# Minys233/GCN-BMP

Hardware: AMD Instinct MI355X
Metric: drug-pairs/sec fwd+bwd, binary-DDI GGNN d=128 (higher is better)
Workload: dtype f32; 1 GPU; C2: full binary DDI set (544 drugs, 147696 pairs), GGNN 4-step d=128 tied + Nie co-attention (head 8, tanh) + MLP(32,16), fwd+bwd+Adam, 1024 pairs/GPU/step, every molecule instance encoded; the 144 batches of one epoch resident in HBM, cycled; layout=per-instance packed layout, whole 128-row tiles, pairs_per_gpu=1024, global_batch=1024, parallelism=dp1

## Files before the change

gcn-bmp_amd/csrc/bmp_coattn.hip:

```cpp
#include <string.h>
#include "bmp_kernels.h"

#define CO_MAXN 128
#define CO_MAXH 16
#define CO_NT_BIG 1024
#define CO_DQ 4
#define CO_NT_FWD 512

struct CoArgs {
    const float* X1; const float* X2;
    const float* Q2;
    const float* Z1; const float* Z2; int ZC;
    const float* w1; const float* w2;
    const int* r1; const int* n1; const int* r2; const int* n2;
    const long long* coff;
    const int* order; int order_off;
    int np;
    const float* wa1; const float* wa2; const float* cbias;
    int d, o, H, act, ldc;
    int mode;
    float* Cbuf;
    float* H1; float* H2;
    float* al1; float* al2;
    float* out1; float* out2;
    const float* dout1; const float* dout2;
    float* dQ2; float* dX1;
    float* dZ1; float* dZ2;
    float* dpart;
    float* big_ws; long long big_stride;
    const int* rm1; const int* rm2; int N1, N2;
    const float* gscale;
};

struct CoLds {
    float* Cs;
    float* dSs;
    float* P1s;
    float* P2s;
    float* dH1s;
    float* dH2s;
    float* w1s; float* w2s; float* v2s;
    float* cmax; float* invD2; float* rmax; float* invD1;
    float* s1; float* s2;
    float* dots1; float* dots2;
    float* H1s; float* H2s;
    float* do1; float* do2;
    float* Up; float* dPp; float* cmb;
};

__device__ __forceinline__ CoLds co_carve(float* base, int np, int ldc, int H, bool bwd, int o = 0, int nt = 256, bool big = false) {
    CoLds L;
    float* p = base;
    L.Cs = p; p += (size_t)np * ldc;
    L.dSs = p; if (bwd) p += (size_t)np * ldc;
    L.P1s = p; p += np * H;
    L.P2s = p; p += np * H;
    L.dH1s = p; if (bwd) p += np * H;
    L.dH2s = p; if (bwd) p += np * H;
    L.w1s = p; p += np;
    L.w2s = p; p += np;
    L.v2s = p; p += np;
    L.cmax = p; p += np; L.invD2 = p; p += np; L.rmax = p; p += np; L.invD1 = p; p += np;
    L.s1 = p; p += np;
    L.s2 = p; p += np;
    L.dots1 = p; p += np; L.dots2 = p; p += np;
    L.H1s = p; if (bwd) p += np * H;
    L.H2s = p; if (bwd) p += np * H;
    L.do1 = p; if (bwd) p += o;
    L.do2 = p; if (bwd) p += o;
    L.cmb = p; if (bwd) p += np;
    if (big) { L.Up = p; if (bwd) p += np; L.dPp = p; if (bwd) p += np * H; }
    else if (np >= 128) { L.Up = L.dots1; L.dPp = L.H1s; }
    else { L.Up = p; if (bwd) p += nt; L.dPp = p; if (bwd) p += nt * H; }
    return L;
}

static size_t co_lds_floats(int np, int ldc, int H, bool bwd, int o = 0, int nt = 256, bool big = false) {
    return (size_t)np * ldc * (bwd ? 2 : 1) + (size_t)np * H * (bwd ? 6 : 2) + 11 * (size_t)np + (bwd ? 2 * (size_t)o + np : 0) +
           (big ? (bwd ? np + np * (size_t)H : 0) : ((bwd && np < 128) ? nt + nt * (size_t)H : 0));
}
static int co_big_np(int np_big) { return (np_big + 31) & ~31; }
static size_t co_big_stride(int np_big, int H, bool bwd, int o) {
    const int np = co_big_np(np_big);
    return (co_lds_floats(np, np + 1, H, bwd, o, 512, true) + 15) & ~(size_t)15;
}

__device__ __forceinline__ void co_stats(const CoLds& L, int n1, int n2, int ldc) {
    const int tid = threadIdx.x;
    if (tid < CO_MAXN) {
        const int j = tid;
        if (j < n1) {
            float mx = -INFINITY;
            for (int i = 0; i < n2; ++i) if (L.w2s[i] > 0.f) mx = fmaxf(mx, L.Cs[i * ldc + j]);
            float s = 0.f;
            for (int i = 0; i < n2; ++i) if (L.w2s[i] > 0.f) s += L.w2s[i] * bmp_exp(L.Cs[i * ldc + j] - mx);
            L.cmax[j] = mx; L.invD2[j] = 1.f / s;
        }
    } else {
        const int i = tid - CO_MAXN;
        if (i < n2) {
            float mx = -INFINITY;
            for (int j = 0; j < n1; ++j) if (L.w1s[j] > 0.f) mx = fmaxf(mx, L.Cs[i * ldc + j]);
            float s = 0.f;
            for (int j = 0; j < n1; ++j) if (L.w1s[j] > 0.f) s += L.w1s[j] * bmp_exp(L.Cs[i * ldc + j] - mx);
            L.rmax[i] = mx; L.invD1[i] = 1.f / s;
        }
    }
}

__device__ __forceinline__ float grp_max(float v, int Q) {
    for (int m = Q >> 1; m >= 1; m >>= 1) v = fmaxf(v, __shfl_xor(v, m));
    return v;
}
__device__ __forceinline__ float grp_sum(float v, int Q) {
    for (int m = Q >> 1; m >= 1; m >>= 1) v += __shfl_xor(v, m);
    return v;
}
__device__ __forceinline__ int co_split(int n1, int n2, int nt) {
    int Q = 1;
    while (Q < 16 && 2 * Q * (n1 + n2) <= nt) Q *= 2;
    return Q;
}
__device__ __forceinline__ void co_stats_split(const CoLds& L, int n1, int n2, int ldc, int Q) {
    const int a = threadIdx.x / Q, q = threadIdx.x % Q;
    if (a < n1) {
        const int j = a;
        float mx = -INFINITY;
        for (int i = q; i < n2; i += Q) if (L.w2s[i] > 0.f) mx = fmaxf(mx, L.Cs[i * ldc + j]);
        mx = grp_max(mx, Q);
        float s = 0.f;
        for (int i = q; i < n2; i += Q) if (L.w2s[i] > 0.f) s += L.w2s[i] * bmp_exp(L.Cs[i * ldc + j] - mx);
        s = grp_sum(s, Q);
        if (q == 0) { L.cmax[j] = mx; L.invD2[j] = 1.f / s; }
    } else if (a < n1 + n2) {
        const int i = a - n1;
        float mx = -INFINITY;
        for (int j = q; j < n1; j += Q) if (L.w1s[j] > 0.f) mx = fmaxf(mx, L.Cs[i * ldc + j]);
        mx = grp_max(mx, Q);
        float s = 0.f;
        for (int j = q; j < n1; j += Q) if (L.w1s[j] > 0.f) s += L.w1s[j] * bmp_exp(L.Cs[i * ldc + j] - mx);
        s = grp_sum(s, Q);
        if (q == 0) { L.rmax[i] = mx; L.invD1[i] = 1.f / s; }
    }
}

__device__ __forceinline__ void co_stats_split_big(const CoLds& L, int n1, int n2, int ldc, int nt) {
    for (int a = threadIdx.x; a < n1 + n2; a += nt) {
        if (a < n1) {
            const int j = a;
            float mx = -INFINITY;
            for (int i = 0; i < n2; ++i) if (L.w2s[i] > 0.f) mx = fmaxf(mx, L.Cs[i * ldc + j]);
            float s = 0.f;
            for (int i = 0; i < n2; ++i) if (L.w2s[i] > 0.f) s += L.w2s[i] * bmp_exp(L.Cs[i * ldc + j] - mx);
            L.cmax[j] = mx; L.invD2[j] = 1.f / s;
        } else {
            const int i = a - n1;
            float mx = -INFINITY;
            for (int j = 0; j < n1; ++j) if (L.w1s[j] > 0.f) mx = fmaxf(mx, L.Cs[i * ldc + j]);
            float s = 0.f;
            for (int j = 0; j < n1; ++j) if (L.w1s[j] > 0.f) s += L.w1s[j] * bmp_exp(L.Cs[i * ldc + j] - mx);
            L.rmax[i] = mx; L.invD1[i] = 1.f / s;
        }
    }
}

__device__ __forceinline__ float co_L2(const CoLds& L, int i, int j, int ldc) {
    return L.w2s[i] > 0.f ? bmp_exp(L.Cs[i * ldc + j] - L.cmax[j]) * L.invD2[j] : 0.f;
}
__device__ __forceinline__ float co_L1(const CoLds& L, int i, int j, int ldc) {
    return L.w1s[j] > 0.f ? bmp_exp(L.Cs[i * ldc + j] - L.rmax[i]) * L.invD1[i] : 0.f;
}

template <int HT, int NT, bool BIG = false>
__global__ __launch_bounds__(NT) void k_coattn_fwd(CoArgs a) {
    constexpr int NW = NT / 64;
    constexpr int HN = HT > 0 ? HT : CO_MAXH;
    extern __shared__ __attribute__((aligned(16))) float lds_raw[];
    const int b = a.order[a.order_off + blockIdx.x];
    const int tid = threadIdx.x, lane = tid & 63, wave = tid >> 6;
    const int l31 = lane & 31, hi = lane >> 5;
    const int r1 = a.r1[b], n1 = a.n1[b], r2 = a.r2[b], n2 = a.n2[b];
    const int d = a.d, o = a.o, H = HT > 0 ? HT : a.H, ZC = a.ZC, ldc = a.ldc;
    const int nb1 = (n1 + 31) >> 5, nb2 = (n2 + 31) >> 5;
    const CoLds L = BIG ? co_carve(a.big_ws + (size_t)blockIdx.x * a.big_stride, a.np, ldc, H, false, 0, NT, true)
                        : co_carve(lds_raw, a.np, ldc, H, false);
    const float cb = a.cbias[0];

    for (int idx = tid; idx < n1 * H; idx += NT) L.P1s[idx] = a.Z1[(size_t)(r1 + idx / H) * ZC + o + idx % H];
    for (int idx = tid; idx < n2 * H; idx += NT) L.P2s[idx] = a.Z2[(size_t)(r2 + idx / H) * ZC + o + idx % H];
    if constexpr (BIG) {
        for (int j = tid; j < n1; j += NT) L.w1s[j] = a.w1[r1 + j];
        for (int i = tid; i < n2; i += NT) { L.w2s[i] = a.w2[r2 + i]; L.v2s[i] = a.Z2[(size_t)(r2 + i) * ZC + o + H]; }
    } else {
    if (tid < n1) L.w1s[tid] = a.w1[r1 + tid];
    if (tid >= CO_MAXN && tid - CO_MAXN < n2) {
        const int i = tid - CO_MAXN;
        L.w2s[i] = a.w2[r2 + i];
        L.v2s[i] = a.Z2[(size_t)(r2 + i) * ZC + o + H];
    }
    }
    __syncthreads();

    for (int blk = wave; blk < nb2 * nb1; blk += NW) {
        const int bi = blk / nb1, bj = blk % nb1;
        int ia = bi * 32 + l31; ia = ia < n2 ? ia : n2 - 1;
        int ja = bj * 32 + l31; ja = ja < n1 ? ja : n1 - 1;
        const float* qa = a.Q2 + (size_t)(r2 + ia) * d + 4 * hi;
        const float* xb = a.X1 + (size_t)(r1 + ja) * d + 4 * hi;
        f32x16 acc;
#pragma unroll
        for (int t = 0; t < 16; ++t) acc[t] = 0.f;
#pragma unroll 8
        for (int k0 = 0; k0 < d; k0 += 8) {
            const f32x4 av = *(const f32x4*)(qa + k0);
            const f32x4 bv = *(const f32x4*)(xb + k0);
#pragma unroll
            for (int t = 0; t < 4; ++t) acc = bmp_mfma(av[t], bv[t], acc);
        }
        const int j = bj * 32 + l31;
        const float v1j = j < n1 ? a.Z1[(size_t)(r1 + j) * ZC + o + H] : 0.f;
        float* cg = a.Cbuf + a.coff[b];
#pragma unroll
        for (int reg = 0; reg < 16; ++reg) {
            const int i = bi * 32 + bmp_acc_row(reg, lane);
            if (i < n2 && j < n1) {
                const float cv = bmp_act(a.act, acc[reg] + v1j + L.v2s[i] + cb);
                L.Cs[i * ldc + j] = cv;
                if (a.Cbuf) cg[(size_t)i * n1 + j] = cv;
            }
        }
    }
    __syncthreads();
    if (a.mode == 1) {
        for (int t_ = tid; t_ < (BIG ? n1 + n2 : NT); t_ += NT) {
        const bool s1 = BIG ? t_ < n1 : t_ < CO_MAXN;
        if (s1) {
            const int j = t_;
            if (j < n1) {
                float s = 0.f, A2 = 0.f;
                for (int i = 0; i < n2; ++i) { s += L.w2s[i] * L.Cs[i * ldc + j]; A2 += L.w2s[i]; }
                L.s1[j] = s / A2;
            }
        } else {
            const int i = t_ - (BIG ? n1 : CO_MAXN);
            if (i < n2) {
                float s = 0.f, A1 = 0.f;
                for (int j = 0; j < n1; ++j) { s += L.w1s[j] * L.Cs[i * ldc + j]; A1 += L.w1s[j]; }
                L.s2[i] = s / A1;
            }
        }
        }
    } else {
    const int Q = BIG ? 1 : co_split(n1, n2, NT);
    if constexpr (BIG) co_stats_split_big(L, n1, n2, ldc, NT);
    else co_stats_split(L, n1, n2, ldc, Q);
    __syncthreads();
    if (a.Cbuf) {
        float* st = a.Cbuf + a.coff[b] + (size_t)n2 * n1;
        if constexpr (BIG) {
            for (int j = tid; j < n1; j += NT) { st[j] = L.cmax[j]; st[n1 + j] = L.invD2[j]; }
            for (int i = tid; i < n2; i += NT) { st[2 * n1 + i] = L.rmax[i]; st[2 * n1 + n2 + i] = L.invD1[i]; }
        } else {
        if (tid < CO_MAXN) { if (tid < n1) { st[tid] = L.cmax[tid]; st[n1 + tid] = L.invD2[tid]; } }
        else if (tid < 2 * CO_MAXN) { const int i = tid - CO_MAXN; if (i < n2) { st[2 * n1 + i] = L.rmax[i]; st[2 * n1 + n2 + i] = L.invD1[i]; } }
        }
    }
    __syncthreads();

    for (int a_ = tid / Q; a_ < (BIG ? n1 + n2 : tid / Q + 1); a_ += NT) {
        const int q = tid % Q;
        const bool side1 = a_ < n1, valid = a_ < n1 + n2;
        const int me = side1 ? a_ : a_ - n1;
        const int no = side1 ? n2 : n1;
        const float* Po = side1 ? L.P2s : L.P1s;
        const float* wo = side1 ? L.w2s : L.w1s;
        float acc[HN];
#pragma unroll
        for (int h = 0; h < HN; ++h) acc[h] = 0.f;
        if (valid) {
            for (int k = q; k < no; k += Q) {
                const float e = wo[k] * (side1 ? co_L1(L, k, me, ldc) : co_L2(L, me, k, ldc));
#pragma unroll
                for (int h = 0; h < HN; ++h) if (h < H) acc[h] += e * Po[k * H + h];
            }
        }
#pragma unroll
        for (int h = 0; h < HN; ++h) if (h < H) acc[h] = grp_sum(acc[h], Q);
        if (valid && q == 0) {
            const float* Pm = side1 ? L.P1s : L.P2s;
            const float* wa = side1 ? a.wa1 : a.wa2;
            float* Hg = a.H1 == nullptr ? nullptr : (side1 ? a.H1 + (size_t)(r1 + me) * H : a.H2 + (size_t)(r2 + me) * H);
            float sc = 0.f;
#pragma unroll
            for (int h = 0; h < HN; ++h) if (h < H) {
                const float hv = bmp_tanh(Pm[me * H + h] + acc[h]);
                if (Hg) Hg[h] = hv;
                sc += hv * wa[h];
            }
            (side1 ? L.s1 : L.s2)[me] = sc;
        }
    }
    }
    __syncthreads();

    if (wave < 2) {
        float* sc = wave == 0 ? L.s1 : L.s2;
        const float* ww = wave == 0 ? L.w1s : L.w2s;
        const int n = wave == 0 ? n1 : n2;
        float mx = -INFINITY;
        for (int k = lane; k < n; k += 64) if (ww[k] > 0.f) mx = fmaxf(mx, sc[k]);
        mx = bmp_wave_max(mx);
        float s = 0.f;
        for (int k = lane; k < n; k += 64) if (ww[k] > 0.f) s += ww[k] * bmp_exp(sc[k] - mx);
        s = bmp_wave_sum(s);
        float* alg = a.al1 == nullptr ? nullptr : (wave == 0 ? a.al1 + r1 : a.al2 + r2);
        for (int k = lane; k < n; k += 64) {
            const float al = ww[k] > 0.f ? bmp_exp(sc[k] - mx) / s : 0.f;
            sc[k] = al;
            if (alg) alg[k] = al;
        }
    }
    __syncthreads();

    {
        constexpr int KG = NT / 256;
        const int kg = tid >> 8, side = (tid >> 7) & 1, t = tid & 127;
        const float* Z = side == 0 ? a.Z1 + (size_t)r1 * ZC : a.Z2 + (size_t)r2 * ZC;
        const float* al = side == 0 ? L.s1 : L.s2;
        const float* ww = side == 0 ? L.w1s : L.w2s;
        const int n = side == 0 ? n1 : n2;
        const int chunk = (n + KG - 1) / KG, k_lo = kg * chunk, k_hi = (k_lo + chunk) < n ? (k_lo + chunk) : n;
        float* out = (side == 0 ? a.out1 : a.out2) + (size_t)b * o;
        float* part = L.Cs;
        for (int c0 = 0; c0 < o; c0 += 128) {
            const int c = c0 + t;
            float acc = 0.f;
            if (c < o) {
#pragma unroll 8
                for (int k = k_lo; k < k_hi; ++k) acc += ww[k] * al[k] * Z[(size_t)k * ZC + c];
            }
            if (KG == 1) {
                if (c < o) out[c] = acc;
            } else {
                __syncthreads();
                part[(kg * 2 + side) * 128 + t] = acc;
                __syncthreads();
                if (kg == 0 && c < o) {
                    float v = part[side * 128 + t];
#pragma unroll
                    for (int g = 1; g < KG; ++g) v += part[(g * 2 + side) * 128 + t];
                    out[c] = v;
                }
            }
        }
    }
}

template <int HT, int NT, bool BIG = false>
__global__ __launch_bounds__(NT) void k_coattn_bwd(CoArgs a) {
    constexpr int NW = NT / 64;
    constexpr int HN = HT > 0 ? HT : CO_MAXH;
    extern __shared__ __attribute__((aligned(16))) float lds_raw[];
    const int b = a.order[a.order_off + blockIdx.x];
    const int tid = threadIdx.x, lane = tid & 63, wave = tid >> 6;
    const int l31 = lane & 31, hi = lane >> 5;
    const int r1 = a.r1[b], n1 = a.n1[b], r2 = a.r2[b], n2 = a.n2[b];
    const int d = a.d, o = a.o, H = HT > 0 ? HT : a.H, ZC = a.ZC, ldc = a.ldc;
    const int nb1 = (n1 + 31) >> 5, nb2 = (n2 + 31) >> 5;
    const int n1p = nb1 * 32, n2p = nb2 * 32;
    const CoLds L = BIG ? co_carve(a.big_ws + (size_t)blockIdx.x * a.big_stride, a.np, ldc, H, true, o, NT, true)
                        : co_carve(lds_raw, a.np, ldc, H, true, o, NT);
    if (a.rm1 != nullptr) {
        for (int row = r1 + n1; row < a.N1 && a.rm1[row] < 0; ++row) {
            for (int c = tid; c < d; c += NT) a.dX1[(size_t)row * d + c] = 0.f;
            for (int c = tid; c < ZC; c += NT) a.dZ1[(size_t)row * ZC + c] = 0.f;
        }
        for (int row = r2 + n2; row < a.N2 && a.rm2[row] < 0; ++row) {
            for (int c = tid; c < d; c += NT) a.dQ2[(size_t)row * d + c] = 0.f;
            for (int c = tid; c < ZC; c += NT) a.dZ2[(size_t)row * ZC + c] = 0.f;
        }
    }
    {
        const float* st = a.Cbuf + a.coff[b] + (size_t)n2 * n1;
        if constexpr (BIG) {
            for (int j = tid; j < n1; j += NT) { L.cmax[j] = st[j]; L.invD2[j] = st[n1 + j]; }
            for (int i = tid; i < n2; i += NT) { L.rmax[i] = st[2 * n1 + i]; L.invD1[i] = st[2 * n1 + n2 + i]; }
        } else {
        if (tid < CO_MAXN) { if (tid < n1) { L.cmax[tid] = st[tid]; L.invD2[tid] = st[n1 + tid]; } }
        else if (tid < 2 * CO_MAXN) { const int i = tid - CO_MAXN; if (i < n2) { L.rmax[i] = st[2 * n1 + i]; L.invD1[i] = st[2 * n1 + n2 + i]; } }
        }
    }
    for (int idx = tid; idx < n1 * H; idx += NT) L.P1s[idx] = a.Z1[(size_t)(r1 + idx / H) * ZC + o + idx % H];
    for (int idx = tid; idx < n2 * H; idx += NT) L.P2s[idx] = a.Z2[(size_t)(r2 + idx / H) * ZC + o + idx % H];
    for (int idx = tid; idx < n1 * H; idx += NT) L.H1s[idx] = a.H1[(size_t)r1 * H + idx];
    for (int idx = tid; idx < n2 * H; idx += NT) L.H2s[idx] = a.H2[(size_t)r2 * H + idx];
    {
        const float gs = a.gscale ? a.gscale[0] : 1.f;
        for (int c = tid; c < o; c += NT) { L.do1[c] = a.dout1[(size_t)b * o + c] * gs; L.do2[c] = a.dout2[(size_t)b * o + c] * gs; }
    }
    if constexpr (BIG) {
        for (int j = tid; j < n1; j += NT) { L.w1s[j] = a.w1[r1 + j]; L.s1[j] = a.al1[r1 + j]; }
        for (int i = tid; i < n2; i += NT) { L.w2s[i] = a.w2[r2 + i]; L.s2[i] = a.al2[r2 + i]; }
    } else {
    if (tid < n1) { L.w1s[tid] = a.w1[r1 + tid]; L.s1[tid] = a.al1[r1 + tid]; }
    if (tid >= CO_MAXN && tid - CO_MAXN < n2) {
        const int i = tid - CO_MAXN;
        L.w2s[i] = a.w2[r2 + i]; L.s2[i] = a.al2[r2 + i];
    }
    }
    {
        const float* cg = a.Cbuf + a.coff[b];
        for (int idx = tid; idx < n2p * ldc; idx += NT) { L.dSs[idx] = 0.f; }
        for (int idx = tid; idx < n2 * n1; idx += NT) L.Cs[(idx / n1) * ldc + idx % n1] = cg[idx];
    }
    const int ncb = (d + 31) >> 5;
    float pre[16];
#pragma unroll
    for (int t = 0; t < 16; ++t) pre[t] = 0.f;
    if (wave < (nb2 + nb1) * ncb) {
        const bool isq = wave < nb2 * ncb;
        const int bc = (isq ? wave : wave - nb2 * ncb) % ncb;
        const int col = bc * 32 + l31;
        const int colc = col < d ? col : d - 1;
        const int kn = isq ? n1 : n2;
        const float* src = isq ? a.X1 + (size_t)r1 * d : a.Q2 + (size_t)r2 * d;
#pragma unroll
        for (int ks = 0; ks < 4; ++ks)
#pragma unroll
            for (int t = 0; t < 4; ++t) {
                const int k = ks * 8 + 4 * hi + t;
                pre[ks * 4 + t] = src[(size_t)(k < kn ? k : kn - 1) * d + colc];
            }
    }

    __syncthreads();

    {
        const int nrows = n1 + n2;
        for (int rbase = wave; rbase < nrows; rbase += CO_DQ * NW) {
            float dot[CO_DQ];
#pragma unroll
            for (int q = 0; q < CO_DQ; ++q) dot[q] = 0.f;
            for (int c = lane; c < o; c += 64) {
                float zq[CO_DQ];
#pragma unroll
                for (int q = 0; q < CO_DQ; ++q) {
                    const int row = rbase + NW * q;
                    const size_t gr = row < n1 ? (size_t)(r1 + row) : (size_t)(r2 + row - n1);
                    zq[q] = row < nrows ? (row < n1 ? a.Z1 : a.Z2)[gr * ZC + c] : 0.f;
                }
#pragma unroll
                for (int q = 0; q < CO_DQ; ++q) {
                    const int row = rbase + NW * q;
                    if (row < nrows) {
                        const bool s1 = row < n1;
                        const int k = s1 ? row : row - n1;
                        const float g = (s1 ? L.do1 : L.do2)[c];
                        const float wa = s1 ? L.w1s[k] * L.s1[k] : L.w2s[k] * L.s2[k];
                        dot[q] += zq[q] * g;
                        (s1 ? a.dZ1 : a.dZ2)[(size_t)(s1 ? r1 + k : r2 + k) * ZC + c] = wa * g;
                    }
                }
            }
#pragma unroll
            for (int q = 0; q < CO_DQ; ++q) {
                const int row = rbase + NW * q;
                const float dsum = bmp_wave_sum(dot[q]);
                if (lane == 0 && row < nrows) (row < n1 ? L.dots1 : L.dots2)[row < n1 ? row : row - n1] = dsum;
            }
        }
    }
    __syncthreads();

    if (wave < 2) {
        const float* al = wave == 0 ? L.s1 : L.s2;
        const float* ww = wave == 0 ? L.w1s : L.w2s;
        float* dt = wave == 0 ? L.dots1 : L.dots2;
        const int n = wave == 0 ? n1 : n2;
        float tsum = 0.f;
        for (int k = lane; k < n; k += 64) tsum += al[k] * ww[k] * dt[k];
        tsum = bmp_wave_sum(tsum);
        for (int k = lane; k < n; k += 64) dt[k] = al[k] * (ww[k] * dt[k] - ww[k] * tsum);
    }
    __syncthreads();
    if (a.mode == 1) {
        float A1 = 0.f, A2 = 0.f;
        for (int j = 0; j < n1; ++j) A1 += L.w1s[j];
        for (int i = 0; i < n2; ++i) A2 += L.w2s[i];
        for (int idx = tid; idx < n2 * n1; idx += NT) {
            const int i = idx / n1, j = idx % n1;
            const float dc = L.w2s[i] / A2 * L.dots1[j] + L.w1s[j] / A1 * L.dots2[i];
            L.dSs[i * ldc + j] = dc * bmp_dact(a.act, L.Cs[i * ldc + j]);
        }
        if (tid < 2 * H) a.dpart[(size_t)b * (2 * H + 1) + tid] = 0.f;
    } else {
    for (int idx = tid; idx < (n1 + n2) * H; idx += NT) {
        const int row = idx / H, h = idx % H;
        const int side = row < n1 ? 0 : 1;
        const int k = side == 0 ? row : row - n1;
        const float hv = (side == 0 ? L.H1s : L.H2s)[k * H + h];
        const float ds = (side == 0 ? L.dots1 : L.dots2)[k];
        const float wa = side == 0 ? a.wa1[h] : a.wa2[h];
        (side == 0 ? L.dH1s : L.dH2s)[k * H + h] = ds * wa * (1.f - hv * hv);
    }
    if (tid < 2 * H) {
        const int side = tid / H, h = tid % H;
        const int n = side == 0 ? n1 : n2;
        float acc = 0.f;
// ... 429 lines not shown
```

gcn-bmp_amd/csrc/bmp_mlp.hip:

```cpp
#include <string.h>
#include "bmp_common.h"
#include "bmp_kernels.h"

#define MLP_MAXL 4
#define MLP_MAXW 64
#define MLP_MAXIN 1024
#define MLP_FR 8
#define MLP_BR 8

struct MlpArgs {
    const float* x1; const float* x2; int d1, d2;
    int B, nl;
    int dims[MLP_MAXL + 1];
    const float* W[MLP_MAXL]; const float* b[MLP_MAXL];
    float* act[MLP_MAXL];
    const float* dy; float* dx1; float* dx2; float* slab; int slab_stride;
};

__global__ __launch_bounds__(256) void k_mlp_fwd(MlpArgs a) {
    __shared__ float buf[2][MLP_FR][MLP_MAXIN];
    extern __shared__ float wt[];
    const int tid = threadIdx.x;
    const int row0 = blockIdx.x * MLP_FR;
    const int in0 = a.dims[0];
// ... 78 lines not shown
    for (int l = a.nl - 1; l >= 0; --l) {
        const int ni = a.dims[l], no = a.dims[l + 1];
        const float* __restrict__ W = a.W[l];
        float* dW = slab + off_l[l];
        if (DW) {
        for (int k = tid; k < ni; k += 256) {
            float xk[MLP_BR];
#pragma unroll
            for (int r = 0; r < MLP_BR; ++r) xk[r] = l == 0 ? xin[r][k] : hid[l - 1][r][k];
#pragma unroll 8
            for (int j = 0; j < no; ++j) {
                float acc = 0.f;
#pragma unroll
                for (int r = 0; r < MLP_BR; ++r) acc += dcur[cur][r][j] * xk[r];
                dW[j * ni + k] = acc;
            }
        }
        for (int j = tid; j < no; j += 256) {
            float acc = 0.f;
            for (int r = 0; r < MLP_BR; ++r) acc += dcur[cur][r][j];
            dW[no * ni + j] = acc;
        }
        }
        if (l > 0) {
            for (int idx = tid; idx < MLP_BR * ni; idx += 256) {
                const int r = idx / ni, k = idx % ni;
                float acc = 0.f;
#pragma unroll 8
                for (int j = 0; j < no; ++j) acc += dcur[cur][r][j] * W[(size_t)j * ni + k];
                dcur[cur ^ 1][r][k] = hid[l - 1][r][k] > 0.f ? acc : 0.f;
            }
        } else if (DX) {
            for (int k = tid; k < ni; k += 256) {
                float acc[MLP_BR];
#pragma unroll
                for (int r = 0; r < MLP_BR; ++r) acc[r] = 0.f;
#pragma unroll 8
                for (int j = 0; j < no; ++j) {
                    const float wv = W[(size_t)j * ni + k];
#pragma unroll
                    for (int r = 0; r < MLP_BR; ++r) acc[r] += dcur[cur][r][j] * wv;
                }
#pragma unroll
                for (int r = 0; r < MLP_BR; ++r) {
                    const int row = row0 + r;
                    if (row >= a.B) continue;
                    if (k < a.d1) a.dx1[(size_t)row * a.d1 + k] = acc[r];
                    else a.dx2[(size_t)row * a.d2 + (k - a.d1)] = acc[r];
                }
            }
        }
        __syncthreads();
        cur ^= 1;
    }
}

struct MlpRedArgs { const float* slab; int nslab, stride; float* dW[MLP_MAXL]; float* db[MLP_MAXL]; int off[MLP_MAXL + 1]; int nw[MLP_MAXL]; int nl;
                    const float* gscale; };
__global__ __launch_bounds__(256) void k_mlp_reduce(MlpRedArgs a) {
    __shared__ float red[4][64];
    const int total = a.off[a.nl];
    const int c = threadIdx.x & 63, g = threadIdx.x >> 6;
    const int i = blockIdx.x * 64 + c;
    float v = 0.f;
    if (i < total)
        for (int s = g; s < a.nslab; s += 4) v += a.slab[(size_t)s * a.stride + i];
    red[g][c] = v;
    __syncthreads();
    if (g == 0 && i < total) {
        v = (red[0][c] + red[1][c]) + (red[2][c] + red[3][c]);
        if (a.gscale) v *= a.gscale[0];
        int l = 0;
        while (l + 1 < a.nl && i >= a.off[l + 1]) ++l;
        const int loc = i - a.off[l];
        if (loc < a.nw[l]) a.dW[l][loc] = v;
        else if (a.db[l]) a.db[l][loc - a.nw[l]] = v;
    }
}

static int mlp_fill(MlpArgs& a, const float* x1, int d1, const float* x2, int d2, int B, int nl, const int* dims,
                    const float* const* W, const float* const* b, float* const* act) {
    memset(&a, 0, sizeof(a));
    BMP_REQUIRE(nl >= 1 && nl <= MLP_MAXL && B > 0 && x1 && d1 > 0 && d2 >= 0 && (d2 == 0 || x2));
    BMP_REQUIRE(dims[0] == d1 + d2 && dims[0] <= MLP_MAXIN);
    for (int l = 0; l < nl; ++l) {
        BMP_REQUIRE(dims[l + 1] > 0 && dims[l + 1] <= MLP_MAXW && W[l] && act[l]);
        a.W[l] = W[l]; a.b[l] = b ? b[l] : nullptr; a.act[l] = act[l];
    }
    for (int l = 0; l <= nl; ++l) a.dims[l] = dims[l];
    a.x1 = x1; a.x2 = x2; a.d1 = d1; a.d2 = d2; a.B = B; a.nl = nl;
    return 0;
}

extern "C" int bmp_mlp_fwd(const float* x1, int d1, const float* x2, int d2, int B, int nl, const int* dims,
                           const float* const* W, const float* const* b, float* const* act, hipStream_t st) {
    MlpArgs a;
    int rc = mlp_fill(a, x1, d1, x2, d2, B, nl, dims, W, b, act);
    if (rc) return rc;
    const size_t wt_bytes = (size_t)dims[0] * (dims[1] + 1) * sizeof(float);
    if (int rc_attr = bmp_lds_attr((const void*)k_mlp_fwd, (size_t)(160 * 1024 - 65536))) return rc_attr;
    BMP_REQUIRE(wt_bytes + 65536 <= 160 * 1024);
    hipLaunchKernelGGL(k_mlp_fwd, dim3((B + MLP_FR - 1) / MLP_FR), dim3(256), wt_bytes, st, a);
    BMP_LAUNCH_CHECK();
    return 0;
}

extern "C" size_t bmp_mlp_bwd_ws_floats(int B, int nl, const int* dims) {
    size_t per = 0;
    for (int l = 0; l < nl; ++l) per += (size_t)dims[l + 1] * (dims[l] + 1);
    return per * ((B + MLP_BR - 1) / MLP_BR);
}

extern "C" int bmp_mlp_bwd(const float* dy, const float* x1, int d1, const float* x2, int d2, int B, int nl, const int* dims,
                           const float* const* W, float* const* act, float* dx1, float* dx2, float* const* dW,
                           float* const* db, float* ws, size_t ws_floats, hipStream_t st, hipStream_t st_w) {
    MlpArgs a;
    int rc = mlp_fill(a, x1, d1, x2, d2, B, nl, dims, W, nullptr, act);
    if (rc) return rc;
    BMP_REQUIRE(dy && dx1 && (d2 == 0 || dx2) && dW && ws && ws_floats >= bmp_mlp_bwd_ws_floats(B, nl, dims));
    const int nwg = (B + MLP_BR - 1) / MLP_BR;
    MlpRedArgs r; memset(&r, 0, sizeof(r));
    int off = 0;
    for (int l = 0; l < nl; ++l) {
        BMP_REQUIRE(dW[l] != nullptr);
        r.off[l] = off; r.nw[l] = dims[l + 1] * dims[l]; r.dW[l] = dW[l]; r.db[l] = db ? db[l] : nullptr;
        off += dims[l + 1] * (dims[l] + 1);
    }
    r.off[nl] = off; r.nl = nl; r.slab = ws; r.nslab = nwg; r.stride = off;
    a.dy = dy; a.dx1 = dx1; a.dx2 = dx2; a.slab = ws; a.slab_stride = off;
    if (!st_w || st_w == st) {
        hipLaunchKernelGGL((k_mlp_bwd<true, true>), dim3(nwg), dim3(256), 0, st, a);
        BMP_LAUNCH_CHECK();
        st_w = st;
    } else {
        if ((rc = bmp_fork_to(st, st_w))) return rc;
        hipLaunchKernelGGL((k_mlp_bwd<true, false>), dim3(nwg), dim3(256), 0, st, a);
        BMP_LAUNCH_CHECK();
        hipLaunchKernelGGL((k_mlp_bwd<false, true>), dim3(nwg), dim3(256), 0, st_w, a);
        BMP_LAUNCH_CHECK();
    }
    hipLaunchKernelGGL(k_mlp_reduce, dim3((off + 63) / 64), dim3(256), 0, st_w, r);
    BMP_LAUNCH_CHECK();
    return 0;
}

struct HeadArgs {
    const int* t;
    float* dy;
    float* part;
    unsigned* ticket;
    float* loss; float* sums;
};

__global__ __launch_bounds__(256) void k_mlp_sce(MlpArgs a, HeadArgs h) {
    __shared__ float xin[MLP_BR][MLP_MAXIN];
    __shared__ float hid[MLP_MAXL][MLP_BR][MLP_MAXW];
    __shared__ float dcur[2][MLP_BR][MLP_MAXW];
    __shared__ float redf[4];
    __shared__ int redi[4];
    __shared__ int last_flag;
    extern __shared__ float wt[];
    const int tid = threadIdx.x, lane = tid & 63, wv = tid >> 6;
    const int row0 = blockIdx.x * MLP_BR;
    const int in0 = a.dims[0], C = a.dims[a.nl];
    int woff[MLP_MAXL];
    {
        int o = a.dims[0] * (a.dims[1] + 1);
        woff[0] = 0;
        for (int l = 1; l < a.nl; ++l) { woff[l] = o; o += a.dims[l + 1] * (a.dims[l] + 1); }
    }
    for (int idx = tid; idx < MLP_BR * in0; idx += 256) {
        const int r = idx / in0, k = idx % in0, row = row0 + r;
        float v = 0.f;
        if (row < a.B) v = k < a.d1 ? a.x1[(size_t)row * a.d1 + k] : a.x2[(size_t)row * a.d2 + (k - a.d1)];
        xin[r][k] = v;
    }
    {
        const int ni = a.dims[0], no = a.dims[1];
        const float* __restrict__ W = a.W[0];
        for (int idx = tid; idx < no * ni; idx += 256) wt[(idx % ni) * (no + 1) + idx / ni] = W[idx];
    }
    for (int l = 1; l < a.nl; ++l) {
        const int ni = a.dims[l], no = a.dims[l + 1];
        const float* __restrict__ W = a.W[l];
        float* wl = wt + woff[l];
        for (int idx = tid; idx < no * ni; idx += 256) wl[(idx / ni) * (ni + 1) + idx % ni] = W[idx];
    }
    int cnt = 0;
    for (int i = tid; i < a.B * C; i += 256) cnt += h.t[i] != -1 ? 1 : 0;
#pragma unroll
    for (int m = 32; m >= 1; m >>= 1) cnt += __shfl_xor(cnt, m);
    if (lane == 0) redi[wv] = cnt;
    __syncthreads();
    const int n_valid = (redi[0] + redi[1]) + (redi[2] + redi[3]);
    const float inv_n = 1.f / (n_valid > 1 ? (float)n_valid : 1.f);
    for (int l = 0; l < a.nl; ++l) {
        const int ni = a.dims[l], no = a.dims[l + 1];
        const float* __restrict__ bb = a.b[l];
        const bool last = l == a.nl - 1;
        for (int idx = tid; idx < MLP_BR * no; idx += 256) {
            const int r = idx / no, j = idx % no;
            float acc = bb ? bb[j] : 0.f;
            if (l == 0) {
                const float* x = xin[r];
                const float* w = wt + j;
#pragma unroll 8
                for (int k = 0; k < ni; ++k) acc += x[k] * w[k * (no + 1)];
            } else {
                const float* x = hid[l - 1][r];
                const float* w = wt + woff[l] + j * (ni + 1);
#pragma unroll 8
                for (int k = 0; k < ni; ++k) acc += x[k] * w[k];
            }
            if (!last) acc = acc > 0.f ? acc : 0.f;
            hid[l][r][j] = acc;
            if (row0 + r < a.B) a.act[l][(size_t)(row0 + r) * no + j] = acc;
        }
        __syncthreads();
    }
    float lsum = 0.f;
    for (int idx = tid; idx < MLP_BR * C; idx += 256) {
        const int r = idx / C, j = idx % C, row = row0 + r;
        float g = 0.f;
        if (row < a.B) {
            const int ti = h.t[(size_t)row * C + j];
            if (ti != -1) {
                const float yi = hid[a.nl - 1][r][j];
                lsum += (yi > 0.f ? yi : 0.f) + log1pf(expf(-fabsf(yi))) - (float)ti * yi;
                g = (1.f / (1.f + expf(-yi)) - (float)ti) * inv_n;
            }
            h.dy[(size_t)row * C + j] = g;
        }
        dcur[0][r][j] = g;
    }
#pragma unroll
    for (int m = 32; m >= 1; m >>= 1) lsum += __shfl_xor(lsum, m);
    if (lane == 0) redf[wv] = lsum;
    __syncthreads();
    if (tid == 0) h.part[blockIdx.x] = (redf[0] + redf[1]) + (redf[2] + redf[3]);
    int cur = 0;
    for (int l = a.nl - 1; l >= 0; --l) {
        const int ni = a.dims[l], no = a.dims[l + 1];
        if (l > 0) {
            const float* wl = wt + woff[l];
            for (int idx = tid; idx < MLP_BR * ni; idx += 256) {
                const int r = idx / ni, k = idx % ni;
                float acc = 0.f;
#pragma unroll 8
                for (int j = 0; j < no; ++j) acc += dcur[cur][r][j] * wl[j * (ni + 1) + k];
                dcur[cur ^ 1][r][k] = hid[l - 1][r][k] > 0.f ? acc : 0.f;
            }
        } else {
            for (int k = tid; k < ni; k += 256) {
                float acc[MLP_BR];
#pragma unroll
                for (int r = 0; r < MLP_BR; ++r) acc[r] = 0.f;
                const float* w = wt + k * (no + 1);
#pragma unroll 8
                for (int j = 0; j < no; ++j) {
                    const float wv0 = w[j];
#pragma unroll
                    for (int r = 0; r < MLP_BR; ++r) acc[r] += dcur[cur][r][j] * wv0;
                }
#pragma unroll
                for (int r = 0; r < MLP_BR; ++r) {
                    const int row = row0 + r;
                    if (row >= a.B) continue;
                    if (k < a.d1) a.dx1[(size_t)row * a.d1 + k] = acc[r];
                    else a.dx2[(size_t)row * a.d2 + (k - a.d1)] = acc[r];
                }
            }
        }
        __syncthreads();
        cur ^= 1;
    }
    if (tid == 0) {
        __threadfence();
        const unsigned tk = atomicAdd(h.ticket, 1u);
        last_flag = tk == gridDim.x - 1;
    }
    __syncthreads();
    if (last_flag && tid == 0) {
        __threadfence();
        float num = 0.f;
        for (unsigned w = 0; w < gridDim.x; ++w) num += __hip_atomic_load(h.part + w, __ATOMIC_RELAXED, __HIP_MEMORY_SCOPE_AGENT);
        h.sums[0] = num; h.sums[1] = (float)n_valid;
        h.loss[0] = num * inv_n;
        *h.ticket = 0u;
    }
}

extern "C" size_t bmp_mlp_sce_ws_floats(int B) { return (size_t)(B + MLP_BR - 1) / MLP_BR; }

extern "C" int bmp_mlp_sce_fwdbwd(const float* x1, int d1, const float* x2, int d2, int B, int nl, const int* dims,
                                  const float* const* W, const float* const* b, float* const* act, const int* t, float* dy,
                                  float* dx1, float* dx2, float* loss, float* sums, float* part, unsigned* ticket,
                                  hipStream_t st) {
    MlpArgs a;
    int rc = mlp_fill(a, x1, d1, x2, d2, B, nl, dims, W, b, act);
    if (rc) return rc;
    BMP_REQUIRE(t && dy && dx1 && (d2 == 0 || dx2) && loss && sums && part && ticket);
    a.dx1 = dx1; a.dx2 = dx2;
    HeadArgs h{t, dy, part, ticket, loss, sums};
    size_t wt_bytes = (size_t)dims[0] * (dims[1] + 1) * sizeof(float);
    for (int l = 1; l < nl; ++l) wt_bytes += (size_t)dims[l + 1] * (dims[l] + 1) * sizeof(float);
    if (int rc_attr = bmp_lds_attr((const void*)k_mlp_sce, (size_t)(160 * 1024 - 49152))) return rc_attr;
    BMP_REQUIRE(wt_bytes + 49152 <= 160 * 1024);
    hipLaunchKernelGGL(k_mlp_sce, dim3((B + MLP_BR - 1) / MLP_BR), dim3(256), wt_bytes, st, a, h);
    BMP_LAUNCH_CHECK();
    return 0;
}

extern "C" int bmp_mlp_bwd_w(const float* dy, const float* x1, int d1, const float* x2, int d2, int B, int nl, const int* dims,
                             const float* const* W, float* const* act, float* const* dW, float* const* db, const float* gscale,
                             float* ws, size_t ws_floats, hipStream_t st) {
    MlpArgs a;
    int rc = mlp_fill(a, x1, d1, x2, d2, B, nl, dims, W, nullptr, act);
    if (rc) return rc;
    BMP_REQUIRE(dy && dW && ws && ws_floats >= bmp_mlp_bwd_ws_floats(B, nl, dims));
    const int nwg = (B + MLP_BR - 1) / MLP_BR;
    MlpRedArgs r; memset(&r, 0, sizeof(r));
    int off = 0;
    for (int l = 0; l < nl; ++l) {
        BMP_REQUIRE(dW[l] != nullptr);
        r.off[l] = off; r.nw[l] = dims[l + 1] * dims[l]; r.dW[l] = dW[l]; r.db[l] = db ? db[l] : nullptr;
        off += dims[l + 1] * (dims[l] + 1);
    }
    r.off[nl] = off; r.nl = nl; r.slab = ws; r.nslab = nwg; r.stride = off; r.gscale = gscale;
    a.dy = dy; a.slab = ws; a.slab_stride = off;
    hipLaunchKernelGGL((k_mlp_bwd<false, true>), dim3(nwg), dim3(256), 0, st, a);
    BMP_LAUNCH_CHECK();
    hipLaunchKernelGGL(k_mlp_reduce, dim3((off + 63) / 64), dim3(256), 0, st, r);
    BMP_LAUNCH_CHECK();
    return 0;
}

__global__ __launch_bounds__(1024) void k_sce_fwd(const float* __restrict__ y, const int* __restrict__ t, int n, float* loss,
                                                  float* sums) {
    __shared__ float s0[16], s1[16];
    float acc = 0.f, cnt = 0.f;
    for (int i = threadIdx.x; i < n; i += 1024) {
        const int ti = t[i];
        if (ti != -1) {
            const float yi = y[i];
            const float sp = (yi > 0.f ? yi : 0.f) + log1pf(expf(-fabsf(yi)));
            acc += sp - (float)ti * yi;
            cnt += 1.f;
        }
    }
#pragma unroll
    for (int m = 32; m >= 1; m >>= 1) { acc += __shfl_xor(acc, m); cnt += __shfl_xor(cnt, m); }
    if ((threadIdx.x & 63) == 0) { s0[threadIdx.x >> 6] = acc; s1[threadIdx.x >> 6] = cnt; }
    __syncthreads();
    if (threadIdx.x == 0) {
        float a0 = 0.f, c0 = 0.f;
#pragma unroll
        for (int w = 0; w < 16; ++w) { a0 += s0[w]; c0 += s1[w]; }
        sums[0] = a0; sums[1] = c0;
        loss[0] = a0 / (c0 > 1.f ? c0 : 1.f);
    }
}

__global__ __launch_bounds__(256) void k_sce_bwd(const float* __restrict__ y, const int* __restrict__ t, int n,
                                                 const float* __restrict__ sums, const float* __restrict__ gout,
                                                 float* __restrict__ dy) {
    const float scale = gout[0] / (sums[1] > 1.f ? sums[1] : 1.f);
    for (int i = blockIdx.x * 256 + threadIdx.x; i < n; i += gridDim.x * 256) {
        const int ti = t[i];
        float g = 0.f;
        if (ti != -1) g = (1.f / (1.f + expf(-y[i])) - (float)ti) * scale;
        dy[i] = g;
    }
}

extern "C" int bmp_sce_fwd(const float* y, const int* t, int n, float* loss, float* sums, hipStream_t st) {
    BMP_REQUIRE(n > 0 && y && t && loss && sums);
    hipLaunchKernelGGL(k_sce_fwd, dim3(1), dim3(1024), 0, st, y, t, n, loss, sums);
    BMP_LAUNCH_CHECK();
    return 0;
}

extern "C" int bmp_sce_bwd(const float* y, const int* t, int n, const float* sums, const float* gout, float* dy,
                           hipStream_t st) {
    BMP_REQUIRE(n > 0 && y && t && sums && gout && dy);
    int blocks = (n + 255) / 256;
    if (blocks > 1024) blocks = 1024;
    hipLaunchKernelGGL(k_sce_bwd, dim3(blocks), dim3(256), 0, st, y, t, n, sums, gout, dy);
    BMP_LAUNCH_CHECK();
    return 0;
}
```

Before: 403,500 pairs/s.

## Parallelize BIG co-attention stats, vectorize MLP loads, and rework ticket reduction

```diff
diff --git a/gcn-bmp_amd/csrc/bmp_coattn.hip b/gcn-bmp_amd/csrc/bmp_coattn.hip
--- a/gcn-bmp_amd/csrc/bmp_coattn.hip
+++ b/gcn-bmp_amd/csrc/bmp_coattn.hip
@@ -121,8 +121,11 @@
     while (Q < 16 && 2 * Q * (n1 + n2) <= nt) Q *= 2;
     return Q;
 }
-__device__ __forceinline__ void co_stats_split(const CoLds& L, int n1, int n2, int ldc, int Q) {
-    const int a = threadIdx.x / Q, q = threadIdx.x % Q;
+template <bool PASSES>
+__device__ __forceinline__ void co_stats_split(const CoLds& L, int n1, int n2, int ldc, int Q, int nt) {
+    const int q = threadIdx.x % Q;
+    int a = threadIdx.x / Q;
+    do {
     if (a < n1) {
         const int j = a;
         float mx = -INFINITY;
@@ -142,27 +145,12 @@
         s = grp_sum(s, Q);
         if (q == 0) { L.rmax[i] = mx; L.invD1[i] = 1.f / s; }
     }
-}
-
-__device__ __forceinline__ void co_stats_split_big(const CoLds& L, int n1, int n2, int ldc, int nt) {
-    for (int a = threadIdx.x; a < n1 + n2; a += nt) {
-        if (a < n1) {
-            const int j = a;
-            float mx = -INFINITY;
-            for (int i = 0; i < n2; ++i) if (L.w2s[i] > 0.f) mx = fmaxf(mx, L.Cs[i * ldc + j]);
-            float s = 0.f;
-            for (int i = 0; i < n2; ++i) if (L.w2s[i] > 0.f) s += L.w2s[i] * bmp_exp(L.Cs[i * ldc + j] - mx);
-            L.cmax[j] = mx; L.invD2[j] = 1.f / s;
-        } else {
-            const int i = a - n1;
-            float mx = -INFINITY;
-            for (int j = 0; j < n1; ++j) if (L.w1s[j] > 0.f) mx = fmaxf(mx, L.Cs[i * ldc + j]);
-            float s = 0.f;
-            for (int j = 0; j < n1; ++j) if (L.w1s[j] > 0.f) s += L.w1s[j] * bmp_exp(L.Cs[i * ldc + j] - mx);
-            L.rmax[i] = mx; L.invD1[i] = 1.f / s;
-        }
-    }
-}
+    if constexpr (!PASSES) break;
+    a += nt / Q;
+    } while (a < n1 + n2);
+}
+
+#define CO_BIG_Q 16
 
 __device__ __forceinline__ float co_L2(const CoLds& L, int i, int j, int ldc) {
     return L.w2s[i] > 0.f ? bmp_exp(L.Cs[i * ldc + j] - L.cmax[j]) * L.invD2[j] : 0.f;
@@ -170,6 +158,23 @@
 __device__ __forceinline__ float co_L1(const CoLds& L, int i, int j, int ldc) {
     return L.w1s[j] > 0.f ? bmp_exp(L.Cs[i * ldc + j] - L.rmax[i]) * L.invD1[i] : 0.f;
 }
+
+#ifdef BMP_PHASE_STAMPS
+#define CO_NSTAMP 12
+#define CO_STAMP_WGS 4096
+__device__ unsigned long long g_co_stamps[CO_NSTAMP * CO_STAMP_WGS];
+#define CO_STAMP(i) do { if (threadIdx.x == 0 && blockIdx.x < CO_STAMP_WGS) \
+    g_co_stamps[blockIdx.x * CO_NSTAMP + (i)] = __builtin_amdgcn_s_memtime(); } while (0)
+#define CO_STAMP_VAL(i, v) do { if (threadIdx.x == 0 && blockIdx.x < CO_STAMP_WGS) \
+    g_co_stamps[blockIdx.x * CO_NSTAMP + (i)] = (v); } while (0)
+extern "C" int bmp_coattn_stamps_read(unsigned long long* out, int nwg) {
+    if (nwg > CO_STAMP_WGS) nwg = CO_STAMP_WGS;
+    return (int)hipMemcpyFromSymbol(out, HIP_SYMBOL(g_co_stamps), sizeof(unsigned long long) * CO_NSTAMP * nwg);
+}
+#else
+#define CO_STAMP(i)
+#define CO_STAMP_VAL(i, v)
+#endif
 
 template <int HT, int NT, bool BIG = false>
 __global__ __launch_bounds__(NT) void k_coattn_fwd(CoArgs a) {
@@ -185,6 +190,9 @@
     const CoLds L = BIG ? co_carve(a.big_ws + (size_t)blockIdx.x * a.big_stride, a.np, ldc, H, false, 0, NT, true)
                         : co_carve(lds_raw, a.np, ldc, H, false);
     const float cb = a.cbias[0];
+    CO_STAMP_VAL(8, __builtin_amdgcn_s_memrealtime());
+    CO_STAMP_VAL(7, (unsigned long long)n1 | ((unsigned long long)n2 << 16));
+    CO_STAMP(0);
 
     for (int idx = tid; idx < n1 * H; idx += NT) L.P1s[idx] = a.Z1[(size_t)(r1 + idx / H) * ZC + o + idx % H];
     for (int idx = tid; idx < n2 * H; idx += NT) L.P2s[idx] = a.Z2[(size_t)(r2 + idx / H) * ZC + o + idx % H];
@@ -200,6 +208,7 @@
     }
     }
     __syncthreads();
+    CO_STAMP(1);
 
     for (int blk = wave; blk < nb2 * nb1; blk += NW) {
         const int bi = blk / nb1, bj = blk % nb1;
@@ -231,6 +240,7 @@
         }
     }
     __syncthreads();
+    CO_STAMP(2);
     if (a.mode == 1) {
         for (int t_ = tid; t_ < (BIG ? n1 + n2 : NT); t_ += NT) {
         const bool s1 = BIG ? t_ < n1 : t_ < CO_MAXN;
@@ -251,9 +261,8 @@
         }
         }
     } else {
-    const int Q = BIG ? 1 : co_split(n1, n2, NT);
-    if constexpr (BIG) co_stats_split_big(L, n1, n2, ldc, NT);
-    else co_stats_split(L, n1, n2, ldc, Q);
+    const int Q = BIG ? CO_BIG_Q : co_split(n1, n2, NT);
+    co_stats_split<BIG>(L, n1, n2, ldc, Q, NT);
     __syncthreads();
     if (a.Cbuf) {
         float* st = a.Cbuf + a.coff[b] + (size_t)n2 * n1;
@@ -266,8 +275,9 @@
         }
     }
     __syncthreads();
-
-    for (int a_ = tid / Q; a_ < (BIG ? n1 + n2 : tid / Q + 1); a_ += NT) {
+    CO_STAMP(3);
+
+    for (int a_ = tid / Q; a_ < (BIG ? n1 + n2 : tid / Q + 1); a_ += (BIG ? NT / Q : NT)) {
         const int q = tid % Q;
         const bool side1 = a_ < n1, valid = a_ < n1 + n2;
         const int me = side1 ? a_ : a_ - n1;
@@ -302,6 +312,7 @@
     }
     }
     __syncthreads();
+    CO_STAMP(4);
 
     if (wave < 2) {
         float* sc = wave == 0 ? L.s1 : L.s2;
@@ -321,6 +332,7 @@
         }
     }
     __syncthreads();
+    CO_STAMP(5);
 
     {
         constexpr int KG = NT / 256;
@@ -354,6 +366,8 @@
             }
         }
     }
+    CO_STAMP(6);
+    CO_STAMP_VAL(9, __builtin_amdgcn_s_memrealtime());
 }
 
 template <int HT, int NT, bool BIG = false>
diff --git a/gcn-bmp_amd/csrc/bmp_mlp.hip b/gcn-bmp_amd/csrc/bmp_mlp.hip
--- a/gcn-bmp_amd/csrc/bmp_mlp.hip
+++ b/gcn-bmp_amd/csrc/bmp_mlp.hip
@@ -254,48 +254,89 @@
     float* loss; float* sums;
 };
 
+#ifdef BMP_PHASE_STAMPS
+#define MLP_NSTAMP 16
+#define MLP_STAMP_WGS 4096
+__device__ unsigned long long g_mlp_stamps[MLP_NSTAMP * MLP_STAMP_WGS];
+#define MLP_STAMP(i) do { if (threadIdx.x == 0 && blockIdx.x < MLP_STAMP_WGS) \
+    g_mlp_stamps[blockIdx.x * MLP_NSTAMP + (i)] = __builtin_amdgcn_s_memtime(); } while (0)
+#define MLP_STAMP_REAL(i) do { if (threadIdx.x == 0 && blockIdx.x < MLP_STAMP_WGS) \
+    g_mlp_stamps[blockIdx.x * MLP_NSTAMP + (i)] = __builtin_amdgcn_s_memrealtime(); } while (0)
+extern "C" int bmp_mlp_stamps_read(unsigned long long* out, int nwg) {
+    if (nwg > MLP_STAMP_WGS) nwg = MLP_STAMP_WGS;
+    return (int)hipMemcpyFromSymbol(out, HIP_SYMBOL(g_mlp_stamps), sizeof(unsigned long long) * MLP_NSTAMP * nwg);
+}
+#else
+#define MLP_STAMP(i)
+#define MLP_STAMP_REAL(i)
+#endif
+
+__device__ __forceinline__ int mlp_counted(int4 v) { return (v.x != -1) + (v.y != -1) + (v.z != -1) + (v.w != -1); }
+
 __global__ __launch_bounds__(256) void k_mlp_sce(MlpArgs a, HeadArgs h) {
-    __shared__ float xin[MLP_BR][MLP_MAXIN];
+    __shared__ __attribute__((aligned(16))) float xin[MLP_BR][MLP_MAXIN];
     __shared__ float hid[MLP_MAXL][MLP_BR][MLP_MAXW];
     __shared__ float dcur[2][MLP_BR][MLP_MAXW];
     __shared__ float redf[4];
     __shared__ int redi[4];
-    __shared__ int last_flag;
-    extern __shared__ float wt[];
+    extern __shared__ __attribute__((aligned(16))) float wt[];
     const int tid = threadIdx.x, lane = tid & 63, wv = tid >> 6;
     const int row0 = blockIdx.x * MLP_BR;
     const int in0 = a.dims[0], C = a.dims[a.nl];
+    MLP_STAMP_REAL(14);
+    MLP_STAMP(0);
     int woff[MLP_MAXL];
     {
-        int o = a.dims[0] * (a.dims[1] + 1);
-        woff[0] = 0;
-        for (int l = 1; l < a.nl; ++l) { woff[l] = o; o += a.dims[l + 1] * (a.dims[l] + 1); }
-    }
-    for (int idx = tid; idx < MLP_BR * in0; idx += 256) {
-        const int r = idx / in0, k = idx % in0, row = row0 + r;
-        float v = 0.f;
-        if (row < a.B) v = k < a.d1 ? a.x1[(size_t)row * a.d1 + k] : a.x2[(size_t)row * a.d2 + (k - a.d1)];
-        xin[r][k] = v;
-    }
-    {
-        const int ni = a.dims[0], no = a.dims[1];
-        const float* __restrict__ W = a.W[0];
-        for (int idx = tid; idx < no * ni; idx += 256) wt[(idx % ni) * (no + 1) + idx / ni] = W[idx];
-    }
-    for (int l = 1; l < a.nl; ++l) {
+        int o = 0;
+        for (int l = 0; l < a.nl; ++l) { woff[l] = o; o += a.dims[l + 1] * (a.dims[l] + 1); }
+    }
+    const int nlab = a.B * C;
+    const bool t_vec = ((uintptr_t)h.t & 15) == 0;
+    const int nlab4 = t_vec ? nlab >> 2 : 0;
+    int4 lab0 = make_int4(-1, -1, -1, -1);
+    if (tid < nlab4) lab0 = ((const int4*)h.t)[tid];
+    if (((a.d1 | a.d2) & 3) == 0 && (((uintptr_t)a.x1 | (uintptr_t)a.x2) & 15) == 0) {
+        const int in4 = in0 >> 2;
+        for (int idx = tid; idx < MLP_BR * in4; idx += 256) {
+            const int r = idx / in4, k = (idx % in4) * 4, row = row0 + r;
+            f32x4 v = {0.f, 0.f, 0.f, 0.f};
+            if (row < a.B) v = k < a.d1 ? *(const f32x4*)(a.x1 + (size_t)row * a.d1 + k) : *(const f32x4*)(a.x2 + (size_t)row * a.d2 + (k - a.d1));
+            *(f32x4*)&xin[r][k] = v;
+        }
+    } else {
+        for (int idx = tid; idx < MLP_BR * in0; idx += 256) {
+            const int r = idx / in0, k = idx % in0, row = row0 + r;
+            float v = 0.f;
+            if (row < a.B) v = k < a.d1 ? a.x1[(size_t)row * a.d1 + k] : a.x2[(size_t)row * a.d2 + (k - a.d1)];
+            xin[r][k] = v;
+        }
+    }
+    for (int l = 0; l < a.nl; ++l) {
         const int ni = a.dims[l], no = a.dims[l + 1];
         const float* __restrict__ W = a.W[l];
         float* wl = wt + woff[l];
-        for (int idx = tid; idx < no * ni; idx += 256) wl[(idx / ni) * (ni + 1) + idx % ni] = W[idx];
-    }
-    int cnt = 0;
-    for (int i = tid; i < a.B * C; i += 256) cnt += h.t[i] != -1 ? 1 : 0;
+        if ((ni & 3) == 0 && ((uintptr_t)W & 15) == 0) {
+            const int ni4 = ni >> 2;
+            for (int idx = tid; idx < no * ni4; idx += 256) {
+                const f32x4 v = ((const f32x4*)W)[idx];
+                float* dst = wl + (idx / ni4) * (ni + 1) + (idx % ni4) * 4;
+                dst[0] = v[0]; dst[1] = v[1]; dst[2] = v[2]; dst[3] = v[3];
+            }
+        } else {
+            for (int idx = tid; idx < no * ni; idx += 256) wl[(idx / ni) * (ni + 1) + idx % ni] = W[idx];
+        }
+    }
+    MLP_STAMP(1);
+    int cnt = mlp_counted(lab0);
+    for (int i = tid + 256; i < nlab4; i += 256) cnt += mlp_counted(((const int4*)h.t)[i]);
+    for (int i = nlab4 * 4 + tid; i < nlab; i += 256) cnt += h.t[i] != -1 ? 1 : 0;
 #pragma unroll
     for (int m = 32; m >= 1; m >>= 1) cnt += __shfl_xor(cnt, m);
     if (lane == 0) redi[wv] = cnt;
     __syncthreads();
     const int n_valid = (redi[0] + redi[1]) + (redi[2] + redi[3]);
     const float inv_n = 1.f / (n_valid > 1 ? (float)n_valid : 1.f);
+    MLP_STAMP(2);
     for (int l = 0; l < a.nl; ++l) {
         const int ni = a.dims[l], no = a.dims[l + 1];
         const float* __restrict__ bb = a.b[l];
@@ -303,14 +344,13 @@
         for (int idx = tid; idx < MLP_BR * no; idx += 256) {
             const int r = idx / no, j = idx % no;
             float acc = bb ? bb[j] : 0.f;
+            const float* w = wt + woff[l] + j * (ni + 1);
             if (l == 0) {
                 const float* x = xin[r];
-                const float* w = wt + j;
-#pragma unroll 8
-                for (int k = 0; k < ni; ++k) acc += x[k] * w[k * (no + 1)];
+#pragma unroll 8
+                for (int k = 0; k < ni; ++k) acc += x[k] * w[k];
             } else {
                 const float* x = hid[l - 1][r];
-                const float* w = wt + woff[l] + j * (ni + 1);
 #pragma unroll 8
                 for (int k = 0; k < ni; ++k) acc += x[k] * w[k];
             }
@@ -319,6 +359,7 @@
             if (row0 + r < a.B) a.act[l][(size_t)(row0 + r) * no + j] = acc;
         }
         __syncthreads();
+        MLP_STAMP(3 + l);
     }
     float lsum = 0.f;
     for (int idx = tid; idx < MLP_BR * C; idx += 256) {
@@ -340,11 +381,12 @@
     if (lane == 0) redf[wv] = lsum;
     __syncthreads();
     if (tid == 0) h.part[blockIdx.x] = (redf[0] + redf[1]) + (redf[2] + redf[3]);
+    MLP_STAMP(7);
     int cur = 0;
     for (int l = a.nl - 1; l >= 0; --l) {
         const int ni = a.dims[l], no = a.dims[l + 1];
+        const float* wl = wt + woff[l];
         if (l > 0) {
-            const float* wl = wt + woff[l];
             for (int idx = tid; idx < MLP_BR * ni; idx += 256) {
                 const int r = idx / ni, k = idx % ni;
                 float acc = 0.f;
@@ -357,10 +399,10 @@
                 float acc[MLP_BR];
 #pragma unroll
                 for (int r = 0; r < MLP_BR; ++r) acc[r] = 0.f;
-                const float* w = wt + k * (no + 1);
+                const float* w = wl + k;
 #pragma unroll 8
                 for (int j = 0; j < no; ++j) {
-                    const float wv0 = w[j];
+                    const float wv0 = w[j * (ni + 1)];
 #pragma unroll
                     for (int r = 0; r < MLP_BR; ++r) acc[r] += dcur[cur][r][j] * wv0;
                 }
@@ -375,21 +417,42 @@
         }
         __syncthreads();
         cur ^= 1;
+        MLP_STAMP(8 + (a.nl - 1 - l));
     }
     if (tid == 0) {
-        __threadfence();
-        const unsigned tk = atomicAdd(h.ticket, 1u);
-        last_flag = tk == gridDim.x - 1;
-    }
-    __syncthreads();
-    if (last_flag && tid == 0) {
-        __threadfence();
+        asm volatile("s_waitcnt vmcnt(0)" ::: "memory");
+        __builtin_amdgcn_fence(__ATOMIC_RELEASE, "agent");
+        asm volatile("s_waitcnt vmcnt(0)" ::: "memory");
+        const unsigned tk = __hip_atomic_fetch_add(h.ticket, 1u, __ATOMIC_RELAXED, __HIP_MEMORY_SCOPE_AGENT);
+        const bool last = tk == gridDim.x - 1;
+        if (last) {
+            __builtin_amdgcn_fence(__ATOMIC_ACQUIRE, "agent");
+            asm volatile("s_waitcnt vmcnt(0)" ::: "memory");
+        }
+        redi[0] = last ? 1 : 0;
+    }
+    __syncthreads();
+    MLP_STAMP(12);
+    if (redi[0]) {
+        float* pl = &xin[0][0];
         float num = 0.f;
-        for (unsigned w = 0; w < gridDim.x; ++w) num += __hip_atomic_load(h.part + w, __ATOMIC_RELAXED, __HIP_MEMORY_SCOPE_AGENT);
-        h.sums[0] = num; h.sums[1] = (float)n_valid;
-        h.loss[0] = num * inv_n;
-        *h.ticket = 0u;
-    }
+        for (unsigned base = 0; base < gridDim.x; base += MLP_BR * MLP_MAXIN) {
+            const unsigned n = gridDim.x - base < MLP_BR * MLP_MAXIN ? gridDim.x - base : MLP_BR * MLP_MAXIN;
+            for (unsigned w = tid; w < n; w += 256)
+                pl[w] = __hip_atomic_load(h.part + base + w, __ATOMIC_RELAXED, __HIP_MEMORY_SCOPE_AGENT);
+            __syncthreads();
+            if (tid == 0)
+                for (unsigned w = 0; w < n; ++w) num += pl[w];
+            __syncthreads();
+        }
+        if (tid == 0) {
+            h.sums[0] = num; h.sums[1] = (float)n_valid;
+            h.loss[0] = num * inv_n;
+            __hip_atomic_store(h.ticket, 0u, __ATOMIC_RELAXED, __HIP_MEMORY_SCOPE_AGENT);
+        }
+    }
+    MLP_STAMP(13);
+    MLP_STAMP_REAL(15);
 }
 
 extern "C" size_t bmp_mlp_sce_ws_floats(int B) { return (size_t)(B + MLP_BR - 1) / MLP_BR; }
@@ -406,9 +469,10 @@
     HeadArgs h{t, dy, part, ticket, loss, sums};
     size_t wt_bytes = (size_t)dims[0] * (dims[1] + 1) * sizeof(float);
     for (int l = 1; l < nl; ++l) wt_bytes += (size_t)dims[l + 1] * (dims[l] + 1) * sizeof(float);
-    if (int rc_attr = bmp_lds_attr((const void*)k_mlp_sce, (size_t)(160 * 1024 - 49152))) return rc_attr;
     BMP_REQUIRE(wt_bytes + 49152 <= 160 * 1024);
-    hipLaunchKernelGGL(k_mlp_sce, dim3((B + MLP_BR - 1) / MLP_BR), dim3(256), wt_bytes, st, a, h);
+    const size_t lds_bytes = wt_bytes + ((size_t)dims[1] * (dims[0] + 1) - (size_t)dims[0] * (dims[1] + 1)) * sizeof(float);
+    if (int rc_attr = bmp_lds_attr((const void*)k_mlp_sce, (size_t)(160 * 1024 - 49152 + 1024))) return rc_attr;
+    hipLaunchKernelGGL(k_mlp_sce, dim3((B + MLP_BR - 1) / MLP_BR), dim3(256), lds_bytes, st, a, h);
     BMP_LAUNCH_CHECK();
     return 0;
 }
```

New measurement: 403,200 pairs/s. No clear change (-0.1%).
